# lucidrains/voicebox-pytorch

Hardware: AMD Instinct MI355X
Metric: mel-frames/sec train-step (fwd+bwd+allreduce+clip+Adam) (higher is better)
Workload: dtype f16/bf16 (fp16 forward operands, bf16 backward operands, fp32 accumulate/master); 1 GPU; VoiceBox dim 512 depth 12 heads 16 unconditional, 8x1024 frames per GPU, train; global_batch=8, seq_len=1024, parallelism=dp1

## Files before the change

include/vbx.h:

```cpp
#ifndef VBX_H
#define VBX_H
#include <stddef.h>
#include <stdint.h>

#ifdef __cplusplus
extern "C" {
#endif

#define VBX_VERSION 1

enum { VBX_OK = 0, VBX_EINVAL = -1, VBX_EUNSUPPORTED = -2, VBX_EWORKSPACE = -3 };

int vbx_version(void);
const char* vbx_last_error(void);
int vbx_check_device(int dev);

enum { VBX_GEMM_NT = 0, VBX_GEMM_NN = 1, VBX_GEMM_TN = 2 };

enum {
  VBX_EPI_BF16 = 0,
  VBX_EPI_F32 = 1,
  VBX_EPI_QKV = 2,
  VBX_EPI_GEGLU = 3,
  VBX_EPI_SPLITK = 4,
// ... 352 lines not shown
  float* dcond;
  int dropout;
  unsigned long long drop_seed;
  const float* ada_table;
  const int* ada_counter;
  int ada_slot;
  int ada_stride;
} vbx_io;

size_t vbx_model_wpack_bytes(const vbx_model* m);
size_t vbx_model_act_bytes(const vbx_model* m);
int vbx_model_pack_weights(const vbx_model* m, void* stream);
int vbx_model_adaln_factors(const vbx_model* m, const float** dada, const float** temb, long* w_off, void** dst_f16);
long vbx_model_sq_partials(const vbx_model* m, long* ranges );
int vbx_model_adam_segments(const vbx_model* m, long n_flat, vbx_adam_seg* out, int max_segs, long* total_blocks);
int vbx_model_forward(const vbx_model* m, const vbx_io* io, void* stream);
int vbx_model_adaln_table(const vbx_model* m, const float* temb, int n, float* ada, void* stream);
int vbx_model_backward_head(const vbx_model* m, const vbx_io* io, const float* gscale, void* stream);
int vbx_model_backward_layer(const vbx_model* m, const vbx_io* io, int layer, void* stream);
int vbx_model_backward_embed(const vbx_model* m, const vbx_io* io, void* stream);
int vbx_wgrad_overlap(int on);
int vbx_wgrad_overlap_forks(void);
int vbx_wgrad_overlap_delay(float side_us, float main_us);

void* vbx_model_debug_ptr(const vbx_model* m, const char* name, int layer);

int vbx_split3_f16(const float* src, long rows, int K, long ld, void* dst_f16, int Kp, void* stream);
int vbx_pack_weight3(const float* src, int src_rows, int src_cols, void* dst_f16, int dst_rows, int dst_cols, int rowmap, int F,
                     void* stream);
int vbx_qknorm_rope_f32(const float* raw, int B, int H, int Np, float qk_scale, const float* q_gamma, const float* k_gamma,
                        const float* rot_cos, const float* rot_sin, float* q32, float* k32, float* v32, void* q16, void* k16,
                        void* qb, void* kb, void* v_bf16, void* v16, float* q_rnorm, float* k_rnorm,
                        float q16_scale ,
                        void* stream);
int vbx_attn_fwd_f32(const float* q, const float* k, const float* v, const uint8_t* mask, float* out32, void* out16, void* out_bf16,
                     float* lse, int B, int H, int Np, float scale, void* stream);
int vbx_attn_fwd_f32_dropout(const float* q, const float* k, const float* v, const uint8_t* mask, float* out32, void* out16,
                             void* out_bf16, float* lse, int B, int H, int Np, float scale, const void* bits_rm, float p, void* stream);
int vbx_geglu_f32(const float* h1, float* g32, void* g16, void* g_bf16, void* h1_bf16, long M, int Fp, void* stream);
int vbx_adaln_proj_f32(const float* temb, const float* w, const float* bias, float* ada, int B, int Th, int J, int group, void* stream);
size_t vbx_model_precise_wpack_bytes(const vbx_model* m);
size_t vbx_model_precise_scratch_bytes(const vbx_model* m);
int vbx_model_pack_weights_precise(const vbx_model* m, void* stream);

typedef struct {
  char label[24];
// ... 14 lines not shown
```

voicebox-pytorch_amd/_lib.py:

```python
import ctypes as C
import os

_HERE = os.path.dirname(os.path.abspath(__file__))
LIB_PATH = os.environ.get("VBX_LIB_PATH") or os.path.join(_HERE, "lib", "libvbx_hip.so")

P, I, L, F = C.c_void_p, C.c_int, C.c_long, C.c_float

VBX_GEMM_NT, VBX_GEMM_NN, VBX_GEMM_TN = 0, 1, 2
VBX_EPI_BF16, VBX_EPI_F32, VBX_EPI_QKV, VBX_EPI_GEGLU, VBX_EPI_SPLITK, VBX_EPI_GELU = 0, 1, 2, 3, 4, 5
VBX_GEMM_KERNEL_GEMM5 = 5


class GemmDesc(C.Structure):
    _fields_ = [
        ("mode", I), ("epilogue", I), ("M", I), ("N", I), ("K", I), ("lda", I), ("ldb", I), ("ldc", I),
        ("A", P), ("B", P), ("C", P), ("bias", P), ("resid", P), ("C2", P), ("splits", I),
        ("Np", I), ("H", I), ("qk_scale", F), ("q_gamma", P), ("k_gamma", P), ("rot_cos", P), ("rot_sin", P),
        ("q16", P), ("k16", P), ("qb", P), ("kb", P), ("v", P), ("q_rnorm", P), ("k_rnorm", P), ("f16", I), ("v16", P), ("C3", P),
        ("q_prescale", F),
    ]


_PROTOS = {
    "vbx_version": [],
    "vbx_check_device": [I],
    "vbx_gemm": [C.POINTER(GemmDesc), P],
    "vbx_gemm_select": [I],
    "vbx_gemm_route": [C.POINTER(GemmDesc)],
    "vbx_gemm5_cu_limit": [I],
    "vbx_prof_enable": [I],
    "vbx_wgrad_overlap": [I],
    "vbx_wgrad_overlap_forks": [],
    "vbx_wgrad_overlap_delay": [F, F],
    "vbx_gemm_tn_splitk_grouped": [C.POINTER(GemmDesc), I, P],
    "vbx_splitk_reduce": [P, I, I, I, P, I, I, I, I, I, I, P],
    "vbx_rmsnorm_fwd": [P, P, P, L, P, P, I, I, I, I, I, P],
    "vbx_rmsnorm_bwd_chunks": [I],
    "vbx_rmsnorm_bwd": [P, P, L, P, P, P, P, P, P, I, I, I, I, I, P],
    "vbx_attn_fwd": [P, P, P, P, P, P, P, I, I, I, F, P],
    "vbx_attn_bwd": [P, P, P, P, P, P, P, I, P, P, P, P, P, P, I, I, I, I, F, P, P],
    "vbx_attn_bwd_fused": [P, P, P, P, P, P, P, I, P, P, P, P, P, P, P, P, P, F, P, I, P, I, I, I, F, P, P],
    "vbx_attn_bwd_select": [I],
    "vbx_attn_bwd_variant": [],
    "vbx_dropout_bits_words": [I],
    "vbx_attn_dropout_bits": [P, P, I, I, C.c_ulonglong, C.c_uint, F, P],
    "vbx_dropout_rows": [P, P, L, I, I, C.c_ulonglong, C.c_uint, F, P],
    "vbx_attn_fwd_dropout": [P, P, P, P, P, P, P, I, I, I, F, P, F, P],
    "vbx_attn_bwd_dropout": [P, P, P, P, P, P, P, I, P, P, P, P, P, P, I, I, I, I, F, P, P, F, P],
    "vbx_attn_bwd_fused_tiles": [I],
    "vbx_attn_bwd_fused_dropout": [P, P, P, P, P, P, P, I, P, P, P, P, P, P, P, P, P, F, P, I, P, I, I, I, F, P, P, P, F, P],
    "vbx_qknorm_rope_bwd": [P, P, P, P, P, P, P, P, P, P, F, P, I, P, I, I, I, F, P],
    "vbx_qknorm_rope_bwd_gpart_rows": [I],
    "vbx_pack_embed_input": [P, P, P, P, P, I, I, I, P],
    "vbx_pack_embed_input_text": [P, P, P, P, P, P, I, P, I, L, P, P, I, I, I, P],
    "vbx_cond_emb_bwd": [P, I, P, I, P, L, P, I, I, I, P],
    "vbx_proj_in_kp": [I],
# ... 170 lines not shown
```

voicebox-pytorch_amd/csrc/runtime.hip:

```cpp
#include "common.hpp"
#include "wgrad_overlap_plan.hpp"
#include <stdlib.h>
#include <algorithm>
#include <string.h>
#include <string>
#include <vector>

namespace {

inline size_t al256(size_t x) { return (x + 255) & ~(size_t)255; }

struct Carver {
  char* base;
  size_t off = 0;
  explicit Carver(void* b) : base((char*)b) {}
  template <class T>
  T* take(size_t n) {
    off = al256(off);
    T* p = base ? (T*)(base + off) : nullptr;
    off += n * sizeof(T);
    return p;
  }
};

struct Dims {
  int B, N, R, Np, D, H, I, F, Fp, Th, L, ks, J, E, Ke, Din;
  int Lc, Kp, Do, Dop;
  long M, M0;
// ... 282 lines not shown
    if (!g_prof.on) return;
    if (g_prof.recs.size() >= 8192) return;
    hipStreamCaptureStatus cs = hipStreamCaptureStatusNone;
    if (hipStreamIsCapturing(st, &cs) != hipSuccess || cs != hipStreamCaptureStatusNone) return;
    ProfRec r{label, nullptr, nullptr};
    if (hipEventCreate(&r.e0) != hipSuccess || hipEventCreate(&r.e1) != hipSuccess) return;
    (void)hipEventRecord(r.e0, st);
    idx = (int)g_prof.recs.size();
    g_prof.recs.push_back(r);
  }
  ~ProfScope() {
    if (idx >= 0) (void)hipEventRecord(g_prof.recs[idx].e1, st);
  }
};

#define CK(x)                 \
  do {                        \
    int rc__ = (x);           \
    if (rc__ != 0) return rc__; \
  } while (0)

struct WgoSide {
  hipStream_t st = nullptr;
  hipEvent_t ev[wgrad_overlap::EV_N] = {};
};
int g_wgo_on = -1;
float g_wgo_delay[2] = {0.f, 0.f};
int g_wgo_forks = 0;
bool wgo_enabled() {
  if (g_wgo_on < 0) {
    const char* e = getenv("VBX_WGRAD_OVERLAP");
    g_wgo_on = e ? (atoi(e) != 0) : 1;
  }
  return g_wgo_on != 0;
}
WgoSide* wgo_side(bool create) {
  static WgoSide* sides[64] = {};
  int dev = 0;
  if (hipGetDevice(&dev) != hipSuccess || dev < 0 || dev >= 64) return nullptr;
  if (sides[dev] || !create) return sides[dev];
  WgoSide* s = new WgoSide;
  int least = 0, greatest = 0;
  const char* pe = getenv("VBX_WGRAD_OVERLAP_PRIORITY");
  const bool low = !(pe && !strcmp(pe, "default"));
  bool ok = hipDeviceGetStreamPriorityRange(&least, &greatest) == hipSuccess &&
            hipStreamCreateWithPriority(&s->st, hipStreamNonBlocking, low ? least : 0) == hipSuccess;
  for (int i = 0; ok && i < wgrad_overlap::EV_N; i++) ok = hipEventCreateWithFlags(&s->ev[i], hipEventDisableTiming) == hipSuccess;
  if (!ok) {
    for (auto e : s->ev) if (e) (void)hipEventDestroy(e);
    if (s->st) (void)hipStreamDestroy(s->st);
    delete s;
    (void)hipGetLastError();
    return nullptr;
  }
  return sides[dev] = s;
}
bool capturing(hipStream_t st) {
  hipStreamCaptureStatus cs = hipStreamCaptureStatusNone;
  return hipStreamIsCapturing(st, &cs) != hipSuccess || cs != hipStreamCaptureStatusNone;
}
int wgo_sync(WgoSide* sd, hipStream_t main_st, wgrad_overlap::Point p, int l, int L) {
  if (!sd) return 0;
  const wgrad_overlap::Sync s = wgrad_overlap::sync_at(p, l, L);
  if (s.kind == wgrad_overlap::SYNC_NONE) return 0;
  hipStream_t st = s.stream == wgrad_overlap::MAIN ? main_st : sd->st;
  const hipError_t e = s.kind == wgrad_overlap::SYNC_RECORD ? hipEventRecord(sd->ev[s.ev], st) : hipStreamWaitEvent(st, sd->ev[s.ev], 0);
  VBX_REQUIRE(e == hipSuccess, "weight-gradient overlap: event %s failed (%s)", s.kind == wgrad_overlap::SYNC_RECORD ? "record" : "wait",
              hipGetErrorString(e));
  return 0;
}
struct WgoGuard {
  WgoSide* sd = nullptr;
  bool forked = false, ok = false;
  int done(int rc) { ok = rc == 0; return rc; }
  ~WgoGuard() {
    if (forked && !ok && sd) (void)hipStreamSynchronize(sd->st);
  }
};
bool defers(const vbx_model* m) { return m->defer_reduce && !m->gateloop && !m->unet && (m->plain_norm || m->adaln_factors); }
struct { const void* act = nullptr; int dxb = 0, dqkv = 0; } g_last_copy;

int check_model(const vbx_model* m) {
  VBX_REQUIRE(m && m->params && m->off && m->wpack && m->act && m->rot_cos && m->rot_sin, "vbx_model: null field");
  VBX_REQUIRE(m->D % 64 == 0 && m->D <= 2048, "vbx_model: dim must be a multiple of 64 and <= 2048 (got %d)", m->D);
  VBX_REQUIRE(m->H > 0 && m->H % 2 == 0, "vbx_model: heads must be even (dim_head is fixed at 64)");
  VBX_REQUIRE(m->Th % 8 == 0 && m->L > 0 && m->B > 0 && m->N > 0 && m->R >= 0 && m->F > 0, "vbx_model: bad dims");
  VBX_REQUIRE(m->ksize >= 1 && m->ksize <= 31 && (m->ksize & 1), "vbx_model: conv_pos_embed_kernel_size must be odd and <= 31 (got %d)", m->ksize);
  VBX_REQUIRE(m->E >= 0 && m->E % 8 == 0 && (m->E == 0 || (m->V1 > 0 && !m->stack_only)), "vbx_model: bad dim_cond_emb / table size");
  const long DT = (long)m->D * m->Th;
  for (int l = 0; l < m->L; l++) {
    const long* o = m->off + VBX_NG + (long)l * VBX_NL;
    if (m->plain_norm) continue;
    VBX_REQUIRE(o[VBX_L_B1W] == o[VBX_L_G1W] + DT && o[VBX_L_G2W] == o[VBX_L_B1W] + DT && o[VBX_L_B2W] == o[VBX_L_G2W] + DT,
                "vbx_model: adaLN weights of layer %d are not contiguous in (g1,b1,g2,b2) order", l);
    VBX_REQUIRE(o[VBX_L_B1B] == o[VBX_L_G1B] + m->D && o[VBX_L_G2B] == o[VBX_L_B1B] + m->D && o[VBX_L_B2B] == o[VBX_L_G2B] + m->D,
                "vbx_model: adaLN biases of layer %d are not contiguous in (g1,b1,g2,b2) order", l);
  }
  for (int l = 0; l < m->L && m->gateloop; l++) {
    const long* o = m->off + VBX_NG + (long)l * VBX_NL;
    VBX_REQUIRE(o[VBX_L_GLLNB] == o[VBX_L_GLLNW] + m->D,
                "vbx_model: GateLoop post-LayerNorm weight and bias of layer %d are not contiguous", l);
  }
// ... 102 lines not shown
      CK(vbx_adaln_proj_f32(temb, P + o[VBX_L_G1W], P + o[VBX_L_G1B], ada + (size_t)l * n * 4 * d.D, n, d.Th, 4 * d.D, 4 * d.D, stream));
    }
    return 0;
  }
  return vbx_adaln_proj_fwd(temb, w.adah, w.bada, ada, n, d.Th, d.J, 4 * d.D, stream);
}

extern "C" int vbx_model_forward(const vbx_model* m, const vbx_io* io, void* stream) {
  CK(check_model(m));
  VBX_REQUIRE(io && io->x, "vbx_model_forward: null io field");
  VBX_REQUIRE(m->stack_only ? ((m->plain_norm || io->cond) && io->pred && !io->target) : (io->cond && (io->times || io->ada_table)),
              "vbx_model_forward: null io field");
  VBX_REQUIRE(!io->target || (io->loss_mask && io->loss), "vbx_model_forward: target needs loss_mask and loss");
  VBX_REQUIRE((io->attn_mask == nullptr) == (io->attn_mask_p == nullptr), "vbx_model_forward: attn_mask and attn_mask_p go together");
  hipStream_t st = (hipStream_t)stream;
  const Dims d = dims_of(m);
  WPack w;
  carve_wpack(m, w);
  Acts a;
  carve_acts(m, a);
  const float* P = m->params;
  const long* G = m->off;
  const bool tr = m->training != 0;

  if (m->precise) {
    std::vector<VbxPreciseLayer> pl(d.L);
    for (int l = 0; l < d.L; l++) {
      const ALayer& y = a.layer[l];
      pl[l] = VbxPreciseLayer{y.hn1, y.q16, y.k16, y.qb, y.kb, y.v, y.vh, y.oh, y.o, y.hn2, y.gh, y.g, tr ? y.h1 : nullptr,
                              y.qrn, y.krn, y.lse, w.layer[l].b1, y.hg, y.glp, y.gls, tr ? y.glh : nullptr, (unsigned*)y.dbr, (unsigned*)y.dbc};
    }
    VbxPreciseActs pa{a.four, a.pre, a.temb, a.ada, a.e, a.pred, a.per_b, a.xs.data(), pl.data(), a.embed_in, a.embed_inh, a.hf};
    return vbx_forward_precise(m, io, &pa, stream);
  }

  if (m->stack_only) {
    CK(vbx_stack_input(io->x, d.R ? P + G[VBX_P_REG] : nullptr, a.xs[0], d.B, d.N, d.R, d.D, stream));
    if (!m->plain_norm) CK(vbx_adaln_proj_fwd(io->cond, w.adah, w.bada, a.ada, d.B, d.Th, d.J, 4 * d.D, stream));
  } else {
  if (io->ada_table) {
    VBX_REQUIRE(!tr && io->ada_counter && io->ada_stride >= 1,
                "vbx_model_forward: ada_table is an inference-only input and needs ada_counter and ada_stride >= 1");
    CK(vbx_ada_select(a.ada, d.L, d.B, 4 * d.D, io->ada_table, io->ada_counter, io->ada_stride, io->ada_slot, stream));
  } else {
  CK(vbx_time_embed_fwd(io->times, P + G[VBX_P_SINW], P + G[VBX_P_T1W], P + G[VBX_P_T1B], a.four, a.pre, a.temb, d.B, d.D,
                        d.Th, stream));
  CK(vbx_adaln_proj_fwd(a.temb, w.adah, w.bada, a.ada, d.B, d.Th, d.J, 4 * d.D, stream));
  }
  if (d.Lc) {
    CK(vbx_proj_in_embed(io->x, io->cond, w.pinh, P + G[VBX_P_PINB], io->cond_mask, io->drop_mask, io->null_cond, a.embed_inh,
                         a.embed_in, a.xcb, d.B, d.N, d.Lc, d.D, d.E, stream));
    if (d.E) {
      VBX_REQUIRE(io->cond_ids && io->T > 0, "vbx_model_forward: a text-conditioned model needs cond_ids");
      CK(vbx_embed_text_cols(io->drop_mask, io->cond_ids, io->T, P + G[VBX_P_CEMB], d.E, io->null_id, a.embed_inh, a.embed_in, d.B,
                             d.N, d.D, d.Ke, stream));
    }
  } else if (d.E) {
    VBX_REQUIRE(io->cond_ids && io->T > 0, "vbx_model_forward: a text-conditioned model needs cond_ids");
    CK(vbx_pack_embed_input_text(io->x, io->cond, io->cond_mask, io->drop_mask, io->null_cond, io->cond_ids, io->T,
                                 P + G[VBX_P_CEMB], d.E, io->null_id, a.embed_inh, a.embed_in, d.B, d.N, d.Din, stream));
  } else {
    CK(vbx_pack_embed_input(io->x, io->cond, io->cond_mask, a.embed_inh, a.embed_in, d.B, d.N, d.Din, stream));
  }
  CK(gemm_nt(a.embed_inh, d.Ke, w.embh, d.Ke, (int)d.M0, d.D, d.Ke, VBX_EPI_F32, a.e, d.D, P + G[VBX_P_EMBB], nullptr,
             nullptr, nullptr, st));
  CK(vbx_convpos_fwd(a.e, P + G[VBX_P_CONVW], P + G[VBX_P_CONVB], io->attn_mask, d.R ? P + G[VBX_P_REG] : nullptr, a.xs[0],
                     d.B, d.N, d.R, d.D, d.ks, stream));
  }

  for (int l = 0; l < d.L; l++) {
    const long* o = m->off + VBX_NG + (long)l * VBX_NL;
    const ALayer& y = a.layer[l];
    const float* ada_l = a.ada + (size_t)l * d.B * 4 * d.D;
    const int S = m->gateloop ? 3 : 2;
    float* x0 = layer_input(m, a, l);
    float* x_in = m->gateloop ? a.xs[S * l + 1] : x0;
    float* x_mid = a.xs[S * l + S - 1];
    float* x_out = a.xs[S * l + S];
    if (m->unet && l >= d.L / 2) {
      CK(vbx_unet_cat(a.xs[S * l], a.xs[S * (d.L - 1 - l)], m->skip_scale, a.cat16, nullptr, d.M, d.D, stream));
      CK(gemm_nt(a.cat16, 2 * d.D, w.layer[l].skwh, 2 * d.D, (int)d.M, d.D, 2 * d.D, VBX_EPI_F32, x0, d.D, P + o[VBX_L_SKB], nullptr,
                 nullptr, nullptr, st));
    }
    if (m->gateloop) {
      CK(vbx_rmsnorm_fwd(x0, P + o[VBX_L_GLG], nullptr, 0, y.hg, y.hgh, d.B, d.Np, 0, d.Np, d.D, stream));
      CK(gemm_nt(y.hgh, d.D, w.layer[l].glwh, d.D, (int)d.M, 3 * d.D, d.D, VBX_EPI_F32, y.glp, 3 * d.D, nullptr, nullptr, nullptr,
                 nullptr, st));
      CK(vbx_gateloop_scan_fwd(y.glp, y.gls, tr ? y.glh : nullptr, d.B, d.Np, d.D, stream));
      CK(vbx_layernorm_fwd(y.gls, P + o[VBX_L_GLLNW], P + o[VBX_L_GLLNB], x0, x_in, d.M, d.D, 1e-5f, stream));
    }
// ... 43 lines not shown
  }
  float* pred = io->pred ? io->pred : a.pred;
  CK(gemm_nt(a.hfh, d.D, w.predh, d.D, (int)d.M0, d.Do, d.D, VBX_EPI_F32, pred, d.Do, nullptr, nullptr, nullptr, nullptr, st));
  if (io->target) CK(vbx_masked_mse_fwd(pred, io->target, io->loss_mask, a.per_b, io->loss, d.B, d.N, d.Do, stream));
  return 0;
}

extern "C" int vbx_model_backward_head(const vbx_model* m, const vbx_io* io, const float* gscale, void* stream) {
  CK(check_model(m));
  VBX_REQUIRE(m->training && m->grads && io && io->target && (m->stack_only || io->loss_mask),
              "vbx_model_backward_head: needs a training forward");
  hipStream_t st = (hipStream_t)stream;
  const Dims d = dims_of(m);
  WPack w;
  carve_wpack(m, w);
  Acts a;
  carve_acts(m, a);
  const float* P = m->params;
  float* Gd = m->grads;
  const long* G = m->off;
  WgoGuard guard;
  guard.sd = capturing(st) ? nullptr : wgo_side(false);
  guard.forked = guard.sd != nullptr;
  CK(wgo_sync(guard.sd, st, wgrad_overlap::PT_HEAD_BEGIN, -1, d.L));
  u16* const dxb = defers(m) ? a.copy[wgrad_overlap::BUF_DXB][wgrad_overlap::dxb_read_copy(d.L - 1)] : a.dxb;
  g_last_copy.act = m->act; g_last_copy.dxb = (int)(dxb != a.dxb ? wgrad_overlap::dxb_read_copy(d.L - 1) : 0);
  if (m->stack_only) {
    CK(vbx_pack_weight(io->target, (int)d.M0, d.D, a.dhn, nullptr, (int)d.M0, d.D, 0, 0, stream));
  } else {
    const float* pred = io->pred ? io->pred : a.pred;
    if (d.Dop != d.Do)
      CK(vbx_masked_mse_bwd_ld(a.pred, d.Dop, io->target, io->loss_mask, a.per_b, gscale, a.dpb, d.B, d.N, d.Do, stream));
    else
      CK(vbx_masked_mse_bwd(pred, io->target, io->loss_mask, a.per_b, gscale, nullptr, a.dpb, d.B, d.N, d.Do, stream));
    CK(wgrad(a.dpb, d.Dop, a.hf, d.D, d.Dop, d.D, d.M0, a.slabs, Gd + G[VBX_P_PREDW], d.Do, d.D, 0, 0, st));
    CK(gemm_nn_bf16(a.dpb, d.Dop, w.pred, d.D, (int)d.M0, d.D, d.Dop, a.dhn, d.D, st));
  }
  if (hipMemsetAsync(a.dx, 0, (size_t)d.M * d.D * sizeof(float), st) != hipSuccess ||
      hipMemsetAsync(dxb, 0, (size_t)d.M * d.D * sizeof(u16), st) != hipSuccess) {
    vbx_set_error("vbx_model_backward_head: memset failed");
    return VBX_EINVAL;
  }
  CK(vbx_rmsnorm_bwd(a.xs[(m->gateloop ? 3 : 2) * d.L], P + G[VBX_P_FNG], 0, a.dhn, nullptr, a.dx, dxb, a.npart, nullptr, d.B, d.Np, d.R, d.N, d.D,
                     stream));
  CK(vbx_reduce_norm_partials(a.npart, a.tmp2d, 0, d.B, vbx_rmsnorm_bwd_chunks(d.N), d.D, 1, stream));
  CK(vbx_sum_rows_f32(a.tmp2d, 1, d.D, Gd + G[VBX_P_FNG], d.D, 0, stream));
  return guard.done(0);
}

struct SqLayout { long off[4], per_layer; };
static SqLayout sq_layout(const Dims& d) {
  SqLayout q;
  const long n[4] = {vbx_splitk_reduce_blocks(d.D, d.Fp), vbx_splitk_reduce_blocks(2 * d.Fp, d.D), vbx_splitk_reduce_blocks(d.D, d.I),
                     vbx_splitk_reduce_blocks(3 * d.I, d.D)};
  q.off[0] = 0;
  for (int i = 1; i < 4; i++) q.off[i] = q.off[i - 1] + n[i - 1];
  q.per_layer = q.off[3] + n[3];
  return q;
}
extern "C" long vbx_model_sq_partials(const vbx_model* m, long* ranges) {
  if (check_model(m) != 0) return 0;
  const Dims d = dims_of(m);
  if (ranges) {
    for (int l = 0; l < d.L; l++) {
      const long* o = m->off + VBX_NG + (long)l * VBX_NL;
      const long lo[4] = {o[VBX_L_QKVW], o[VBX_L_OUTW], o[VBX_L_FF1W], o[VBX_L_FF2W]};
      const long sz[4] = {3L * d.I * d.D, (long)d.D * d.I, 2L * d.F * d.D, (long)d.D * d.F};
      for (int i = 0; i < 4; i++) {
        if (i && lo[i] < lo[i - 1] + sz[i - 1]) return 0;
// ... 123 lines not shown
  float* const npart2 = a.npart2 + rr * a.np_stride;
  float* const cpart = a.cpart + rr * a.cp_stride;
  float* const gpart = a.gpart + rr * a.gp_stride;
  float* const csl = pl.defer ? a.cs_layers + rr * a.cs_stride : a.cs_scratch;
  vbx_skr_jobs wj{};
  WgradGroup wgg;
  WgradGroup* wgp = group_wgrad() ? &wgg : nullptr;
  const int gs = wgp ? wgrad_splits3(d) : 0;
  namespace wgo = wgrad_overlap;
  auto copy_of = [&](wgo::Buf b) { return pl.defer ? a.copy[b][wgo::write_copy(b, l)] : a.copy[b][0]; };
  u16* const dxb_in = pl.defer ? a.copy[wgo::BUF_DXB][wgo::dxb_read_copy(l)] : a.dxb;
  u16* const dxb_out = copy_of(wgo::BUF_DXB);
  u16* const dh1 = copy_of(wgo::BUF_DH1);
  u16* const dqkv = copy_of(wgo::BUF_DQKV);
  u16* dxb_attn = wgp ? copy_of(wgo::BUF_DXB2) : dxb_in;
  g_last_copy.act = m->act; g_last_copy.dxb = pl.defer ? wgo::write_copy(wgo::BUF_DXB, l) : 0; g_last_copy.dqkv = pl.defer ? wgo::write_copy(wgo::BUF_DQKV, l) : 0;
  const bool cap = capturing(st);
  const bool fork = pl.defer && wgp && wgo_enabled() && !g_prof.on && !cap;
  WgoGuard guard;
  guard.sd = cap ? nullptr : wgo_side(fork);
  VBX_REQUIRE(!fork || guard.sd, "vbx_model_backward_layer: could not create the weight-gradient side stream");
  if (fork && g_wgo_delay[1] > 0.f) CK(vbx_stream_delay(g_wgo_delay[1], stream));
  CK(wgo_sync(guard.sd, st, wgo::PT_LAYER_BEGIN, l, d.L));
  float* const slabs = fork ? a.slabs_side : a.slabs;
  const size_t sfl = a.slab_floats;
  const SqLayout sql = sq_layout(d);
  float* const sqb = m->sq_partials ? m->sq_partials + (long)l * sql.per_layer : nullptr;
  auto sq_at = [&](int i) { return sqb ? sqb + sql.off[i] : nullptr; };

  { ProfScope ps("dgrad ff_out", st); CK(gemm_nn_bf16(dxb_in, d.D, wl.w2, d.Fp, M, d.Fp, d.D, a.dg, d.Fp, st)); }
  CK(wgrad(dxb_in, d.D, y.g, d.Fp, d.D, d.Fp, d.M, slabs, Gd + o[VBX_L_FF2W], d.D, d.F, 0, 0, st, &wj, wgp, gs, sq_at(0)));
  if (drop_on && m->ff_dropout > 0.f)
    CK(vbx_dropout_rows(nullptr, a.dg, d.M, d.Fp, d.Fp, io->drop_seed, 2u * l + 1u, m->ff_dropout, stream));
  CK(vbx_geglu_bwd_colsum(y.h1, a.dg, dh1, M, d.Fp, csl, stream));
  { ProfScope ps("dgrad ff_in", st); CK(gemm_nn_bf16(dh1, 2 * d.Fp, wl.w1, d.D, M, d.D, 2 * d.Fp, a.dhn, d.D, st)); }
  CK(wgrad(dh1, 2 * d.Fp, y.hn2, d.D, 2 * d.Fp, d.D, d.M, slabs + sfl, Gd + o[VBX_L_FF1W], 2 * d.F, d.D, 1, d.F, st, &wj, wgp, gs, sq_at(1)));
  CK(vbx_rmsnorm_bwd(x_mid, g2, gstride, a.dhn, a.dx, a.dx, dxb_attn, npart, cpart, d.B, d.Np, 0, d.Np, d.D, stream));

  { ProfScope ps("dgrad to_out", st); CK(gemm_nn_bf16(dxb_attn, d.D, wl.out, d.I, M, d.I, d.D, a.dO, d.I, st)); }
  CK(wgrad(dxb_attn, d.D, y.o, d.I, d.D, d.I, d.M, slabs + 2 * sfl, Gd + o[VBX_L_OUTW], d.D, d.I, 0, 0, st, &wj, wgp, gs, sq_at(2)));
  { ProfScope ps("bwd attention", st);
    CK(vbx_attn_bwd_fused_dropout(y.q16, y.k16, y.qb, y.kb, y.v, attn_mask_p, y.oh, 1, a.dO, y.lse, a.delta, y.qrn, y.krn, q_gamma, k_gamma,
                                  m->rot_cos, m->rot_sin, m->qk_norm ? 8.0f : 0.0f, dqkv, 3 * d.I, gpart, d.B, d.H, d.Np, m->attn_scale,
                                  a.attn_scratch, drop_on ? y.dbr : nullptr, y.dbc, m->attn_dropout, stream)); }
  { ProfScope ps("dgrad to_qkv", st); CK(gemm_nn_bf16(dqkv, 3 * d.I, wl.qkv, d.D, M, d.D, 3 * d.I, a.dhn, d.D, st)); }
  CK(wgrad(dqkv, 3 * d.I, y.hn1, d.D, 3 * d.I, d.D, d.M, slabs + 3 * sfl, Gd + o[VBX_L_QKVW], 3 * d.I, d.D, 0, 0, st, &wj, wgp, gs, sq_at(3)));

  if (fork) {
    hipStream_t side = guard.sd->st;
    CK(wgo_sync(guard.sd, st, wgo::PT_FORK, l, d.L));
    guard.forked = true;
    g_wgo_forks++;
    CK(wgo_sync(guard.sd, st, wgo::PT_SIDE_BEGIN, l, d.L));
    if (g_wgo_delay[0] > 0.f) CK(vbx_stream_delay(g_wgo_delay[0], side));
    if (wgg.n) CK(vbx_gemm_tn_splitk_grouped(wgg.d, wgg.n, side));
    CK(wgo_sync(guard.sd, st, wgo::PT_SIDE_GEMM_DONE, l, d.L));
    if (wj.n) CK(vbx_splitk_reduce_multi(&wj, side));
    CK(wgo_sync(guard.sd, st, wgo::PT_SIDE_REDUCE_DONE, l, d.L));
  } else {
    if (wgg.n) { ProfScope ps("wgrad (4 GEMMs)", st); CK(vbx_gemm_tn_splitk_grouped(wgg.d, wgg.n, stream)); }
    if (wj.n) { ProfScope ps("wgrad slab reduce", st); CK(vbx_splitk_reduce_multi(&wj, stream)); }
  }
  CK(vbx_rmsnorm_bwd(x_in, g1, gstride, a.dhn, a.dx, a.dx, dxb_out, npart2, nullptr, d.B, d.Np, 0, d.Np, d.D, stream));

  vbx_mr_jobs jb{};
  if (!pl.defer) {
    layer_reduce_jobs(m, d, a, pl, l, 0, jb);
    CK(vbx_multi_reduce(&jb, stream));
  } else if (l == 0) {
    ProfScope ps("partials reduce (all)", st);
    for (int ll = d.L - 1; ll >= 0; ll--) {
      layer_reduce_jobs(m, d, a, pl, ll, ll, jb);
      if (jb.n + 8 > VBX_MR_MAX || ll == 0) {
        CK(vbx_multi_reduce(&jb, stream));
        jb.n = 0;
      }
    }
  }

  if (m->gateloop) CK(backward_gateloop(m, d, w, a, l, stream));
  if (m->unet) CK(backward_unet(m, d, w, a, l, stream));
  if (m->plain_norm) return guard.done(0);
  if (pl.ada_all) {
    if (l == 0) {
      ProfScope ps("adaLN dtemb (all)", st);
      CK(vbx_adaln_dtemb_all(w.adah, a.dada, a.dtemb, a.ada_scratch, d.L, d.B, d.Th, 4 * d.D, stream));
    }
    return guard.done(0);
  }
  return guard.done(vbx_adaln_proj_bwd(m->stack_only ? io->cond : a.temb, w.adah + (size_t)l * 4 * d.D * d.Th, dada_l,
                            m->adaln_factors ? nullptr : Gd + o[VBX_L_G1W], Gd + o[VBX_L_G1B], a.dtemb,
                            a.ada_scratch, d.B, d.Th, 4 * d.D, l == d.L - 1 ? 0 : 1, stream));
}

extern "C" int vbx_model_backward_embed(const vbx_model* m, const vbx_io* io, void* stream) {
  CK(check_model(m));
  VBX_REQUIRE(m->training && m->grads && io && (m->stack_only ? io->dx != nullptr : io->times != nullptr),
              "vbx_model_backward_embed: needs a training forward");
  hipStream_t st = (hipStream_t)stream;
  const Dims d = dims_of(m);
  WPack w;
  carve_wpack(m, w);
  Acts a;
  carve_acts(m, a);
  const float* P = m->params;
  float* Gd = m->grads;
  const long* G = m->off;
// ... 103 lines not shown
  carve_acts(m, a);
  if (dada) *dada = a.dada;
  if (temb) *temb = a.temb;
  for (int l = 0; l < d.L; l++) {
    if (w_off) w_off[l] = (m->off + VBX_NG + (long)l * VBX_NL)[VBX_L_G1W];
    if (dst_f16) dst_f16[l] = w.adah + (size_t)l * 4 * d.D * d.Th;
  }
  return d.L;
}

extern "C" int vbx_wgrad_overlap(int on) {
  VBX_REQUIRE(on == 0 || on == 1, "vbx_wgrad_overlap: 0 in line, 1 on the side stream");
  g_wgo_on = on;
  return 0;
}
extern "C" int vbx_wgrad_overlap_forks(void) { return g_wgo_forks; }
extern "C" int vbx_wgrad_overlap_delay(float side_us, float main_us) {
  VBX_REQUIRE(side_us >= 0.f && side_us <= 2000.f && main_us >= 0.f && main_us <= 2000.f, "vbx_wgrad_overlap_delay: 0 .. 2000 us each");
  g_wgo_delay[0] = side_us;
  g_wgo_delay[1] = main_us;
  return 0;
}

extern "C" int vbx_prof_enable(int on) {
  for (auto& r : g_prof.recs) { (void)hipEventDestroy(r.e0); (void)hipEventDestroy(r.e1); }
  g_prof.recs.clear();
  g_prof.on = on != 0;
  return 0;
}
extern "C" int vbx_prof_collect(vbx_prof_entry* out, int max_entries) {
  VBX_REQUIRE(out && max_entries > 0, "vbx_prof_collect: bad args");
  g_prof.on = false;
  int n = 0;
  for (auto& r : g_prof.recs) {
    float ms = 0.f;
    if (hipEventSynchronize(r.e1) != hipSuccess || hipEventElapsedTime(&ms, r.e0, r.e1) != hipSuccess) continue;
    int k = 0;
    for (; k < n; k++)
      if (!strncmp(out[k].label, r.label, sizeof(out[k].label) - 1)) break;
    if (k == n) {
      if (n == max_entries) continue;
      memset(&out[n], 0, sizeof(out[n]));
      strncpy(out[n].label, r.label, sizeof(out[n].label) - 1);
      n++;
    }
    out[k].calls++;
// ... 31 lines not shown
```

Measured before the change: 939,500 mel-frames/s.

## Overlap forward adaLN, head wgrad, memsets and partial reductions on side stream

Extends the side-stream overlap beyond layer weight gradients. The forward time embedding and adaLN projections now run on the side stream while the embed branch runs on main. In backward, the head's to_pred wgrad, the dx/dxb memsets and the final-norm gamma reductions move to the side stream, and deferred per-layer partial reductions are spread across layers on the side stream instead of being done all at layer 0. This is meant to hide small serial kernels behind the main chain, at the cost of extra event syncs, added dependency tracking and a global map of reduction state keyed by activation buffer.

```diff
diff --git a/include/vbx.h b/include/vbx.h
--- a/include/vbx.h
+++ b/include/vbx.h
@@ -398,6 +398,14 @@
 int vbx_wgrad_overlap(int on);
 int vbx_wgrad_overlap_forks(void);
 int vbx_wgrad_overlap_delay(float side_us, float main_us);
+#define VBX_STEP_OVERLAP_FWD 1
+#define VBX_STEP_OVERLAP_HEAD 2
+#define VBX_STEP_OVERLAP_PARTIALS 4
+#define VBX_STEP_OVERLAP_MEMSET 8
+int vbx_step_overlap(int on);
+int vbx_step_overlap_parts(int parts);
+int vbx_step_overlap_forks(void);
+int vbx_step_overlap_plan_forks(int L, int forward);
 
 void* vbx_model_debug_ptr(const vbx_model* m, const char* name, int layer);
 
diff --git a/voicebox-pytorch_amd/_lib.py b/voicebox-pytorch_amd/_lib.py
--- a/voicebox-pytorch_amd/_lib.py
+++ b/voicebox-pytorch_amd/_lib.py
@@ -32,6 +32,10 @@
     "vbx_wgrad_overlap": [I],
     "vbx_wgrad_overlap_forks": [],
     "vbx_wgrad_overlap_delay": [F, F],
+    "vbx_step_overlap": [I],
+    "vbx_step_overlap_parts": [I],
+    "vbx_step_overlap_forks": [],
+    "vbx_step_overlap_plan_forks": [I, I],
     "vbx_gemm_tn_splitk_grouped": [C.POINTER(GemmDesc), I, P],
     "vbx_splitk_reduce": [P, I, I, I, P, I, I, I, I, I, I, P],
     "vbx_rmsnorm_fwd": [P, P, P, L, P, P, I, I, I, I, I, P],
diff --git a/voicebox-pytorch_amd/csrc/runtime.hip b/voicebox-pytorch_amd/csrc/runtime.hip
--- a/voicebox-pytorch_amd/csrc/runtime.hip
+++ b/voicebox-pytorch_amd/csrc/runtime.hip
@@ -1,9 +1,11 @@
 #include "common.hpp"
+#include "step_overlap_plan.hpp"
 #include "wgrad_overlap_plan.hpp"
 #include <stdlib.h>
 #include <algorithm>
 #include <string.h>
 #include <string>
+#include <unordered_map>
 #include <vector>
 
 namespace {
@@ -332,7 +334,7 @@
 
 struct WgoSide {
   hipStream_t st = nullptr;
-  hipEvent_t ev[wgrad_overlap::EV_N] = {};
+  hipEvent_t ev[step_overlap::EV_N] = {};
 };
 int g_wgo_on = -1;
 float g_wgo_delay[2] = {0.f, 0.f};
@@ -355,7 +357,7 @@
   const bool low = !(pe && !strcmp(pe, "default"));
   bool ok = hipDeviceGetStreamPriorityRange(&least, &greatest) == hipSuccess &&
             hipStreamCreateWithPriority(&s->st, hipStreamNonBlocking, low ? least : 0) == hipSuccess;
-  for (int i = 0; ok && i < wgrad_overlap::EV_N; i++) ok = hipEventCreateWithFlags(&s->ev[i], hipEventDisableTiming) == hipSuccess;
+  for (int i = 0; ok && i < step_overlap::EV_N; i++) ok = hipEventCreateWithFlags(&s->ev[i], hipEventDisableTiming) == hipSuccess;
   if (!ok) {
     for (auto e : s->ev) if (e) (void)hipEventDestroy(e);
     if (s->st) (void)hipStreamDestroy(s->st);
@@ -388,6 +390,30 @@
   }
 };
 bool defers(const vbx_model* m) { return m->defer_reduce && !m->gateloop && !m->unet && (m->plain_norm || m->adaln_factors); }
+int g_sto_on = -1;
+int g_sto_parts = -1;
+int g_sto_forks = 0;
+int sto_parts() {
+  if (g_sto_on < 0) {
+    const char* e = getenv("VBX_STEP_OVERLAP");
+    g_sto_on = e ? (atoi(e) != 0) : 1;
+  }
+  if (g_sto_parts < 0) {
+    const char* e = getenv("VBX_STEP_OVERLAP_PARTS");
+    g_sto_parts = e ? (atoi(e) & step_overlap::PART_ALL) : step_overlap::kDefaultParts;
+  }
+  return g_sto_on && wgo_enabled() ? g_sto_parts : 0;
+}
+int sto_sync(WgoSide* sd, hipStream_t main_st, step_overlap::Point p, int l, int L, int parts) {
+  if (!sd) return 0;
+  const step_overlap::Sync s = step_overlap::sync_at(p, l, L, parts);
+  if (s.kind == wgrad_overlap::SYNC_NONE) return 0;
+  hipStream_t st = s.stream == wgrad_overlap::MAIN ? main_st : sd->st;
+  const hipError_t e = s.kind == wgrad_overlap::SYNC_RECORD ? hipEventRecord(sd->ev[s.ev], st) : hipStreamWaitEvent(st, sd->ev[s.ev], 0);
+  VBX_REQUIRE(e == hipSuccess, "step overlap: event %s failed (%s)", s.kind == wgrad_overlap::SYNC_RECORD ? "record" : "wait", hipGetErrorString(e));
+  return 0;
+}
+std::unordered_map<const void*, int> g_sto_reduced;
 struct { const void* act = nullptr; int dxb = 0, dqkv = 0; } g_last_copy;
 
 int check_model(const vbx_model* m) {
@@ -536,6 +562,17 @@
   const float* P = m->params;
   const long* G = m->off;
   const bool tr = m->training != 0;
+  namespace sto = step_overlap;
+  const bool fwd_cap = tr ? capturing(st) : true;
+  const int fwd_parts = (tr && !fwd_cap && !m->stack_only && !m->precise && !m->gateloop && !m->unet && !io->ada_table && !g_prof.on) ? sto_parts() : 0;
+  const bool fwd_fork = sto::has(fwd_parts, sto::PART_FWD);
+  WgoGuard guard;
+  guard.sd = fwd_cap ? nullptr : wgo_side(fwd_fork);
+  VBX_REQUIRE(!fwd_fork || guard.sd, "vbx_model_forward: could not create the side stream");
+  if (fwd_parts) {
+    if (fwd_fork && g_wgo_delay[1] > 0.f) CK(vbx_stream_delay(g_wgo_delay[1], stream));
+    CK(sto_sync(guard.sd, st, sto::PT_FWD_BEGIN_JOIN, -1, d.L, fwd_parts));
+  }
 
   if (m->precise) {
     std::vector<VbxPreciseLayer> pl(d.L);
@@ -557,9 +594,18 @@
                 "vbx_model_forward: ada_table is an inference-only input and needs ada_counter and ada_stride >= 1");
     CK(vbx_ada_select(a.ada, d.L, d.B, 4 * d.D, io->ada_table, io->ada_counter, io->ada_stride, io->ada_slot, stream));
   } else {
+  void* const ada_stream = fwd_fork ? (void*)guard.sd->st : stream;
+  if (fwd_fork) {
+    CK(sto_sync(guard.sd, st, sto::PT_FWD_BEGIN, -1, d.L, fwd_parts));
+    guard.forked = true;
+    g_sto_forks++;
+    CK(sto_sync(guard.sd, st, sto::PT_FWD_SIDE_BEGIN, -1, d.L, fwd_parts));
+    if (g_wgo_delay[0] > 0.f) CK(vbx_stream_delay(g_wgo_delay[0], ada_stream));
+  }
   CK(vbx_time_embed_fwd(io->times, P + G[VBX_P_SINW], P + G[VBX_P_T1W], P + G[VBX_P_T1B], a.four, a.pre, a.temb, d.B, d.D,
-                        d.Th, stream));
-  CK(vbx_adaln_proj_fwd(a.temb, w.adah, w.bada, a.ada, d.B, d.Th, d.J, 4 * d.D, stream));
+                        d.Th, ada_stream));
+  CK(vbx_adaln_proj_fwd(a.temb, w.adah, w.bada, a.ada, d.B, d.Th, d.J, 4 * d.D, ada_stream));
+  if (fwd_fork) CK(sto_sync(guard.sd, st, sto::PT_FWD_SIDE_DONE, -1, d.L, fwd_parts));
   }
   if (d.Lc) {
     CK(vbx_proj_in_embed(io->x, io->cond, w.pinh, P + G[VBX_P_PINB], io->cond_mask, io->drop_mask, io->null_cond, a.embed_inh,
@@ -580,6 +626,10 @@
              nullptr, nullptr, st));
   CK(vbx_convpos_fwd(a.e, P + G[VBX_P_CONVW], P + G[VBX_P_CONVB], io->attn_mask, d.R ? P + G[VBX_P_REG] : nullptr, a.xs[0],
                      d.B, d.N, d.R, d.D, d.ks, stream));
+  }
+  if (fwd_fork) {
+    CK(sto_sync(guard.sd, st, sto::PT_FWD_JOIN, -1, d.L, fwd_parts));
+    guard.forked = false;
   }
 
   for (int l = 0; l < d.L; l++) {
@@ -669,9 +719,29 @@
   WgoGuard guard;
   guard.sd = capturing(st) ? nullptr : wgo_side(false);
   guard.forked = guard.sd != nullptr;
+  namespace sto = step_overlap;
+  const bool cap = capturing(st);
+  const int parts = (defers(m) && !m->stack_only && group_wgrad() && !g_prof.on && !cap) ? sto_parts() : 0;
+  const bool fork = sto::has(parts, sto::PART_HEAD), zero_side = sto::has(parts, sto::PART_HEAD | sto::PART_MEMSET);
+  if (fork) {
+    guard.sd = wgo_side(true);
+    guard.forked = true;
+    VBX_REQUIRE(guard.sd, "vbx_model_backward_head: could not create the side stream");
+    if (g_wgo_delay[1] > 0.f) CK(vbx_stream_delay(g_wgo_delay[1], stream));
+  }
+  hipStream_t const side = fork ? guard.sd->st : st;
+  g_sto_reduced[m->act] = d.L;
   CK(wgo_sync(guard.sd, st, wgrad_overlap::PT_HEAD_BEGIN, -1, d.L));
   u16* const dxb = defers(m) ? a.copy[wgrad_overlap::BUF_DXB][wgrad_overlap::dxb_read_copy(d.L - 1)] : a.dxb;
   g_last_copy.act = m->act; g_last_copy.dxb = (int)(dxb != a.dxb ? wgrad_overlap::dxb_read_copy(d.L - 1) : 0);
+  auto zero_dx = [&](hipStream_t on) {
+    if (hipMemsetAsync(a.dx, 0, (size_t)d.M * d.D * sizeof(float), on) != hipSuccess ||
+        hipMemsetAsync(dxb, 0, (size_t)d.M * d.D * sizeof(u16), on) != hipSuccess) {
+      vbx_set_error("vbx_model_backward_head: memset failed");
+      return (int)VBX_EINVAL;
+    }
+    return 0;
+  };
   if (m->stack_only) {
     CK(vbx_pack_weight(io->target, (int)d.M0, d.D, a.dhn, nullptr, (int)d.M0, d.D, 0, 0, stream));
   } else {
@@ -680,18 +750,33 @@
       CK(vbx_masked_mse_bwd_ld(a.pred, d.Dop, io->target, io->loss_mask, a.per_b, gscale, a.dpb, d.B, d.N, d.Do, stream));
     else
       CK(vbx_masked_mse_bwd(pred, io->target, io->loss_mask, a.per_b, gscale, nullptr, a.dpb, d.B, d.N, d.Do, stream));
-    CK(wgrad(a.dpb, d.Dop, a.hf, d.D, d.Dop, d.D, d.M0, a.slabs, Gd + G[VBX_P_PREDW], d.Do, d.D, 0, 0, st));
+    if (fork) {
+      CK(sto_sync(guard.sd, st, sto::PT_HEAD_FORK, -1, d.L, parts));
+      g_sto_forks++;
+      CK(sto_sync(guard.sd, st, sto::PT_HEAD_SIDE_BEGIN, -1, d.L, parts));
+      if (g_wgo_delay[0] > 0.f) CK(vbx_stream_delay(g_wgo_delay[0], side));
+      if (zero_side) {
+        CK(zero_dx(side));
+        CK(sto_sync(guard.sd, st, sto::PT_HEAD_SIDE_ZERO, -1, d.L, parts));
+      }
+    }
+    CK(wgrad(a.dpb, d.Dop, a.hf, d.D, d.Dop, d.D, d.M0, fork ? a.slabs_side : a.slabs, Gd + G[VBX_P_PREDW], d.Do, d.D, 0, 0, side));
     CK(gemm_nn_bf16(a.dpb, d.Dop, w.pred, d.D, (int)d.M0, d.D, d.Dop, a.dhn, d.D, st));
   }
-  if (hipMemsetAsync(a.dx, 0, (size_t)d.M * d.D * sizeof(float), st) != hipSuccess ||
-      hipMemsetAsync(dxb, 0, (size_t)d.M * d.D * sizeof(u16), st) != hipSuccess) {
-    vbx_set_error("vbx_model_backward_head: memset failed");
-    return VBX_EINVAL;
-  }
+  if (zero_side) CK(sto_sync(guard.sd, st, sto::PT_HEAD_ZERO_JOIN, -1, d.L, parts));
+  else CK(zero_dx(st));
   CK(vbx_rmsnorm_bwd(a.xs[(m->gateloop ? 3 : 2) * d.L], P + G[VBX_P_FNG], 0, a.dhn, nullptr, a.dx, dxb, a.npart, nullptr, d.B, d.Np, d.R, d.N, d.D,
                      stream));
-  CK(vbx_reduce_norm_partials(a.npart, a.tmp2d, 0, d.B, vbx_rmsnorm_bwd_chunks(d.N), d.D, 1, stream));
-  CK(vbx_sum_rows_f32(a.tmp2d, 1, d.D, Gd + G[VBX_P_FNG], d.D, 0, stream));
+  if (fork) {
+    CK(sto_sync(guard.sd, st, sto::PT_HEAD_NORM, -1, d.L, parts));
+    CK(sto_sync(guard.sd, st, sto::PT_HEAD_SIDE_NORM, -1, d.L, parts));
+  }
+  CK(vbx_reduce_norm_partials(a.npart, a.tmp2d, 0, d.B, vbx_rmsnorm_bwd_chunks(d.N), d.D, 1, side));
+  CK(vbx_sum_rows_f32(a.tmp2d, 1, d.D, Gd + G[VBX_P_FNG], d.D, 0, side));
+  if (fork) {
+    CK(sto_sync(guard.sd, st, sto::PT_HEAD_SIDE_DONE, -1, d.L, parts));
+    CK(sto_sync(guard.sd, st, sto::PT_HEAD_SIDE_JOIN, -1, d.L, parts));
+  }
   return guard.done(0);
 }
 
@@ -861,6 +946,12 @@
   VBX_REQUIRE(!fork || guard.sd, "vbx_model_backward_layer: could not create the weight-gradient side stream");
   if (fork && g_wgo_delay[1] > 0.f) CK(vbx_stream_delay(g_wgo_delay[1], stream));
   CK(wgo_sync(guard.sd, st, wgo::PT_LAYER_BEGIN, l, d.L));
+  namespace sto = step_overlap;
+  const int parts = sto_parts();
+  CK(sto_sync(guard.sd, st, sto::PT_LAYER0_BEGIN, l, d.L, parts));
+  auto red = g_sto_reduced.find(m->act);
+  if (red == g_sto_reduced.end() || l == d.L - 1) red = g_sto_reduced.insert_or_assign(m->act, d.L).first;
+  int& reduced_from = red->second;
   float* const slabs = fork ? a.slabs_side : a.slabs;
   const size_t sfl = a.slab_floats;
   const SqLayout sql = sq_layout(d);
@@ -892,6 +983,19 @@
     g_wgo_forks++;
     CK(wgo_sync(guard.sd, st, wgo::PT_SIDE_BEGIN, l, d.L));
     if (g_wgo_delay[0] > 0.f) CK(vbx_stream_delay(g_wgo_delay[0], side));
+    if (sto::has(parts, sto::PART_PARTIALS) && reduced_from > l + 1) {
+      vbx_mr_jobs sj{};
+      for (int ll = reduced_from - 1; ll > l; ll--) {
+        layer_reduce_jobs(m, d, a, pl, ll, ll, sj);
+        if (sj.n + 8 > VBX_MR_MAX || ll == l + 1) {
+          CK(vbx_multi_reduce(&sj, side));
+          sj.n = 0;
+        }
+      }
+      reduced_from = l + 1;
+      g_sto_forks++;
+      CK(sto_sync(guard.sd, st, sto::PT_SIDE_PARTIALS_DONE, l, d.L, parts));
+    }
     if (wgg.n) CK(vbx_gemm_tn_splitk_grouped(wgg.d, wgg.n, side));
     CK(wgo_sync(guard.sd, st, wgo::PT_SIDE_GEMM_DONE, l, d.L));
     if (wj.n) CK(vbx_splitk_reduce_multi(&wj, side));
@@ -908,7 +1012,7 @@
     CK(vbx_multi_reduce(&jb, stream));
   } else if (l == 0) {
     ProfScope ps("partials reduce (all)", st);
-    for (int ll = d.L - 1; ll >= 0; ll--) {
+    for (int ll = reduced_from - 1; ll >= 0; ll--) {
       layer_reduce_jobs(m, d, a, pl, ll, ll, jb);
       if (jb.n + 8 > VBX_MR_MAX || ll == 0) {
         CK(vbx_multi_reduce(&jb, stream));
@@ -922,6 +1026,7 @@
   if (m->plain_norm) return guard.done(0);
   if (pl.ada_all) {
     if (l == 0) {
+      if (reduced_from < d.L) CK(sto_sync(guard.sd, st, sto::PT_DTEMB_BEGIN, l, d.L, sto::PART_PARTIALS));
       ProfScope ps("adaLN dtemb (all)", st);
       CK(vbx_adaln_dtemb_all(w.adah, a.dada, a.dtemb, a.ada_scratch, d.L, d.B, d.Th, 4 * d.D, stream));
     }
@@ -1071,6 +1176,22 @@
   return 0;
 }
 
+extern "C" int vbx_step_overlap(int on) {
+  VBX_REQUIRE(on == 0 || on == 1, "vbx_step_overlap: 0 in line, 1 beside the main chain");
+  g_sto_on = on;
+  return 0;
+}
+extern "C" int vbx_step_overlap_parts(int parts) {
+  VBX_REQUIRE(parts >= -1 && parts <= step_overlap::PART_ALL, "vbx_step_overlap_parts: a mask of VBX_STEP_OVERLAP_* bits, or -1 for the default");
+  g_sto_parts = parts < 0 ? step_overlap::kDefaultParts : parts;
+  return 0;
+}
+extern "C" int vbx_step_overlap_forks(void) { return g_sto_forks; }
+extern "C" int vbx_step_overlap_plan_forks(int L, int forward) {
+  const int parts = sto_parts();
+  return forward ? step_overlap::forward_forks(parts) : step_overlap::backward_forks(L, parts);
+}
+
 extern "C" int vbx_prof_enable(int on) {
   for (auto& r : g_prof.recs) { (void)hipEventDestroy(r.e0); (void)hipEventDestroy(r.e1); }
   g_prof.recs.clear();
diff --git a/voicebox-pytorch_amd/csrc/step_overlap_plan.hpp b/voicebox-pytorch_amd/csrc/step_overlap_plan.hpp
--- /dev/null
+++ b/voicebox-pytorch_amd/csrc/step_overlap_plan.hpp
@@ -0,0 +1,228 @@
+#pragma once
+#include <cstring>
+#include <initializer_list>
+
+#include "wgrad_overlap_plan.hpp"
+
+namespace step_overlap {
+
+namespace wgo = wgrad_overlap;
+using wgo::MAIN;
+using wgo::SIDE;
+using wgo::Stream;
+using wgo::SyncKind;
+
+enum Part { PART_FWD = 1, PART_HEAD = 2, PART_PARTIALS = 4, PART_MEMSET = 8, PART_ALL = 15 };
+constexpr int kDefaultParts = PART_FWD | PART_HEAD | PART_PARTIALS | PART_MEMSET;
+
+enum Event {
+  EV_FWD_BEGIN = wgo::EV_N,
+  EV_ADA,
+  EV_HEAD_FORK,
+  EV_HEAD_ZERO,
+  EV_HEAD_NORM,
+  EV_HEAD_DONE,
+  EV_PARTIALS,
+  EV_N
+};
+
+enum Point {
+  PT_FWD_BEGIN_JOIN,
+  PT_FWD_BEGIN,
+  PT_FWD_SIDE_BEGIN,
+  PT_FWD_SIDE_DONE,
+  PT_FWD_JOIN,
+  PT_HEAD_FORK,
+  PT_HEAD_SIDE_BEGIN,
+  PT_HEAD_SIDE_ZERO,
+  PT_HEAD_ZERO_JOIN,
+  PT_HEAD_NORM,
+  PT_HEAD_SIDE_NORM,
+  PT_HEAD_SIDE_DONE,
+  PT_HEAD_SIDE_JOIN,
+  PT_LAYER0_BEGIN,
+  PT_SIDE_PARTIALS_DONE,
+  PT_DTEMB_BEGIN,
+};
+struct Sync {
+  SyncKind kind;
+  Stream stream;
+  int ev;
+};
+constexpr Sync kNoSync{wgo::SYNC_NONE, MAIN, EV_N};
+constexpr bool has(int parts, int p) { return (parts & p) == p; }
+constexpr Sync sync_at(Point p, int l, int L, int parts) {
+  const bool fwd = has(parts, PART_FWD), head = has(parts, PART_HEAD), zero = has(parts, PART_HEAD | PART_MEMSET);
+  const bool partials = has(parts, PART_PARTIALS) && L >= 2;
+  switch (p) {
+    case PT_FWD_BEGIN_JOIN: return parts ? Sync{wgo::SYNC_WAIT, MAIN, wgo::EV_JOIN} : kNoSync;
+    case PT_FWD_BEGIN: return fwd ? Sync{wgo::SYNC_RECORD, MAIN, EV_FWD_BEGIN} : kNoSync;
+    case PT_FWD_SIDE_BEGIN: return fwd ? Sync{wgo::SYNC_WAIT, SIDE, EV_FWD_BEGIN} : kNoSync;
+    case PT_FWD_SIDE_DONE: return fwd ? Sync{wgo::SYNC_RECORD, SIDE, EV_ADA} : kNoSync;
+    case PT_FWD_JOIN: return fwd ? Sync{wgo::SYNC_WAIT, MAIN, EV_ADA} : kNoSync;
+    case PT_HEAD_FORK: return head ? Sync{wgo::SYNC_RECORD, MAIN, EV_HEAD_FORK} : kNoSync;
+    case PT_HEAD_SIDE_BEGIN: return head ? Sync{wgo::SYNC_WAIT, SIDE, EV_HEAD_FORK} : kNoSync;
+    case PT_HEAD_SIDE_ZERO: return zero ? Sync{wgo::SYNC_RECORD, SIDE, EV_HEAD_ZERO} : kNoSync;
+    case PT_HEAD_ZERO_JOIN: return zero ? Sync{wgo::SYNC_WAIT, MAIN, EV_HEAD_ZERO} : kNoSync;
+    case PT_HEAD_NORM: return head ? Sync{wgo::SYNC_RECORD, MAIN, EV_HEAD_NORM} : kNoSync;
+    case PT_HEAD_SIDE_NORM: return head ? Sync{wgo::SYNC_WAIT, SIDE, EV_HEAD_NORM} : kNoSync;
+    case PT_HEAD_SIDE_DONE: return head ? Sync{wgo::SYNC_RECORD, SIDE, EV_HEAD_DONE} : kNoSync;
+    case PT_HEAD_SIDE_JOIN: return head ? Sync{wgo::SYNC_RECORD, SIDE, wgo::EV_JOIN} : kNoSync;
+    case PT_LAYER0_BEGIN: return head && l == 0 && wgo::last_reader(0, L) < 0 ? Sync{wgo::SYNC_WAIT, MAIN, EV_HEAD_DONE} : kNoSync;
+    case PT_SIDE_PARTIALS_DONE: return partials && l + 1 < L ? Sync{wgo::SYNC_RECORD, SIDE, EV_PARTIALS} : kNoSync;
+    case PT_DTEMB_BEGIN: return partials && l == 0 ? Sync{wgo::SYNC_WAIT, MAIN, EV_PARTIALS} : kNoSync;
+  }
+  return kNoSync;
+}
+constexpr int forward_forks(int parts) { return has(parts, PART_FWD) ? 1 : 0; }
+constexpr int backward_forks(int L, int parts) { return (has(parts, PART_HEAD) ? 1 : 0) + (has(parts, PART_PARTIALS) ? L - 1 : 0); }
+
+enum ResKind {
+  RES_TIME = 100,
+  RES_ADA,
+  RES_DPB,
+  RES_DX,
+  RES_PARTIALS,
+  RES_TMP2D,
+  RES_DADA,
+  RES_GRAD_SMALL,
+  RES_DTEMB,
+  RES_GRAD_TIME,
+};
+struct Res {
+  int kind, a, b;
+};
+struct Op {
+  enum Type { LAUNCH, SYNC } type;
+  Stream stream;
+  const char* name;
+  int layer;
+  Sync sync;
+  bool is_new;
+  Res reads[10], writes[6];
+  int nr, nw;
+};
+inline Op from_wgo(const wgo::Op& w) {
+  Op o{};
+  o.type = w.type == wgo::Op::SYNC ? Op::SYNC : Op::LAUNCH;
+  o.stream = w.stream; o.name = w.name; o.layer = w.layer;
+  o.sync = Sync{w.sync.kind, w.sync.stream, (int)w.sync.ev};
+  for (int i = 0; i < w.nr; i++) o.reads[o.nr++] = Res{(int)w.reads[i].kind, w.reads[i].a, w.reads[i].b};
+  for (int i = 0; i < w.nw; i++) o.writes[o.nw++] = Res{(int)w.writes[i].kind, w.writes[i].a, w.writes[i].b};
+  return o;
+}
+template <class F>
+inline void put_sync(Point p, int l, int L, int parts, F&& f) {
+  const Sync s = sync_at(p, l, L, parts);
+  if (s.kind == wgo::SYNC_NONE) return;
+  Op o{};
+  o.type = Op::SYNC; o.stream = s.stream; o.name = s.kind == wgo::SYNC_WAIT ? "wait" : "record"; o.layer = l; o.sync = s; o.is_new = true;
+  f(o);
+}
+template <class F>
+inline void put_launch(Stream st, const char* name, int l, std::initializer_list<Res> reads, std::initializer_list<Res> writes, F&& f) {
+  Op o{};
+  o.type = Op::LAUNCH; o.stream = st; o.name = name; o.layer = l;
+  for (const Res& r : reads) o.reads[o.nr++] = r;
+  for (const Res& w : writes) o.writes[o.nw++] = w;
+  f(o);
+}
+
+constexpr Res kActs{wgo::RES_FWD_ACTS, 0, 0}, kTime{RES_TIME, 0, 0}, kAda{RES_ADA, 0, 0}, kDpb{RES_DPB, 0, 0}, kDx{RES_DX, 0, 0};
+constexpr Res kTmp2d{RES_TMP2D, 0, 0}, kDtemb{RES_DTEMB, 0, 0}, kSlabsSide{wgo::RES_SLABS_SIDE, 0, 0}, kSlabsMain{wgo::RES_SLABS_MAIN, 0, 0};
+constexpr Res kGradHead{wgo::RES_GRAD_HEAD, 0, 0}, kGradEmbed{wgo::RES_GRAD_EMBED, 0, 0}, kGradTime{RES_GRAD_TIME, 0, 0};
+constexpr Res partials(int region) { return Res{RES_PARTIALS, region, 0}; }
+constexpr Res dada(int l) { return Res{RES_DADA, l, 0}; }
+constexpr Res grad_small(int l) { return Res{RES_GRAD_SMALL, l, 0}; }
+
+template <class F>
+inline void emit_forward(int L, int parts, F&& f) {
+  const Stream ada_on = has(parts, PART_FWD) ? SIDE : MAIN;
+  put_sync(PT_FWD_BEGIN_JOIN, -1, L, parts, f);
+  put_sync(PT_FWD_BEGIN, -1, L, parts, f);
+  put_sync(PT_FWD_SIDE_BEGIN, -1, L, parts, f);
+  put_launch(ada_on, "time embedding", -1, {}, {kTime}, f);
+  put_launch(ada_on, "adaLN projections", -1, {kTime}, {kAda}, f);
+  put_sync(PT_FWD_SIDE_DONE, -1, L, parts, f);
+  put_launch(MAIN, "embed branch (pack, to_embed, conv)", -1, {}, {kActs}, f);
+  put_sync(PT_FWD_JOIN, -1, L, parts, f);
+  for (int l = 0; l < L; l++) put_launch(MAIN, "forward layer", l, {kAda, kActs}, {kActs}, f);
+  put_launch(MAIN, "final norm, to_pred, loss", -1, {kActs}, {kActs}, f);
+}
+
+template <class F>
+inline void emit_head(int L, int parts, F&& f) {
+  const bool head = has(parts, PART_HEAD), zero = has(parts, PART_HEAD | PART_MEMSET);
+  const Res dxb{wgo::RES_BUF, wgo::BUF_DXB, wgo::dxb_read_copy(L - 1)};
+  wgo::emit_sync(wgo::PT_HEAD_BEGIN, -1, L, [&](const wgo::Op& o) { f(from_wgo(o)); });
+  put_launch(MAIN, "mse backward", -1, {kActs}, {kDpb}, f);
+  put_sync(PT_HEAD_FORK, -1, L, parts, f);
+  put_sync(PT_HEAD_SIDE_BEGIN, -1, L, parts, f);
+  if (zero) put_launch(SIDE, "memsets (dx, dxb)", -1, {}, {kDx, dxb}, f);
+  put_sync(PT_HEAD_SIDE_ZERO, -1, L, parts, f);
+  put_launch(head ? SIDE : MAIN, "to_pred wgrad + reduce", -1, {kDpb, kActs}, {head ? kSlabsSide : kSlabsMain, kGradHead}, f);
+  put_launch(MAIN, "dgrad to_pred", -1, {kDpb}, {}, f);
+  if (!zero) put_launch(MAIN, "memsets (dx, dxb)", -1, {}, {kDx, dxb}, f);
+  put_sync(PT_HEAD_ZERO_JOIN, -1, L, parts, f);
+  put_launch(MAIN, "final norm backward", -1, {kActs}, {kDx, dxb, partials(0)}, f);
+  put_sync(PT_HEAD_NORM, -1, L, parts, f);
+  put_sync(PT_HEAD_SIDE_NORM, -1, L, parts, f);
+  put_launch(head ? SIDE : MAIN, "final norm gamma: reduce partials", -1, {partials(0)}, {kTmp2d}, f);
+  put_launch(head ? SIDE : MAIN, "final norm gamma: sum rows", -1, {kTmp2d}, {kGradHead}, f);
+  put_sync(PT_HEAD_SIDE_DONE, -1, L, parts, f);
+  put_sync(PT_HEAD_SIDE_JOIN, -1, L, parts, f);
+}
+
+template <class F>
+inline void emit_layer(int l, int L, int parts, F&& f) {
+  const bool partials_side = has(parts, PART_PARTIALS);
+  put_sync(PT_LAYER0_BEGIN, l, L, parts, f);
+  wgo::emit_layer(l, L, [&](const wgo::Op& w) {
+    Op o = from_wgo(w);
+    if (w.type == wgo::Op::LAUNCH && w.stream == MAIN) {
+      const bool norm = !strncmp(w.name, "norm backward", 13);
+      if (norm) { o.reads[o.nr++] = kAda; o.reads[o.nr++] = kDx; o.writes[o.nw++] = kDx; }
+      if (norm || !strcmp(w.name, "GEGLU backward") || !strcmp(w.name, "attention backward")) o.writes[o.nw++] = partials(l);
+    }
+    f(o);
+    if (w.type == wgo::Op::SYNC && w.point == wgo::PT_SIDE_BEGIN && partials_side && l + 1 < L) {
+      put_launch(SIDE, "partials reduce", l + 1, {partials(l + 1)}, {dada(l + 1), grad_small(l + 1)}, f);
+      put_sync(PT_SIDE_PARTIALS_DONE, l, L, parts, f);
+    }
+  });
+  if (l != 0) return;
+  for (int ll = L - 1; ll >= 0; ll--)
+    if (ll == 0 || !partials_side) put_launch(MAIN, "partials reduce", ll, {partials(ll)}, {dada(ll), grad_small(ll)}, f);
+  put_sync(PT_DTEMB_BEGIN, 0, L, parts, f);
+  Op o{};
+  o.type = Op::LAUNCH; o.stream = MAIN; o.name = "adaLN dtemb (all)"; o.layer = -1;
+  o.reads[o.nr++] = dada(0);
+  o.writes[o.nw++] = kDtemb;
+  f(o);
+}
+
+template <class F>
+inline void emit_embed(int L, int parts, F&& f) {
+  (void)parts;
+  put_launch(MAIN, "conv backward + finalize", -1, {kDx, kActs}, {kGradEmbed}, f);
+  wgo::emit_embed(L, [&](const wgo::Op& w) {
+    if (w.type == wgo::Op::SYNC) {
+      put_launch(MAIN, "time MLP backward", -1, {kDtemb, kTime}, {kGradTime}, f);
+    }
+    f(from_wgo(w));
+  });
+}
+
+template <class F>
+inline void emit_backward(int L, int parts, F&& f) {
+  emit_head(L, parts, f);
+  for (int l = L - 1; l >= 0; l--) emit_layer(l, L, parts, f);
+  emit_embed(L, parts, f);
+}
+template <class F>
+inline void emit_step(int L, int parts, F&& f) {
+  emit_forward(L, parts, f);
+  emit_backward(L, parts, f);
+}
+
+}
```

New measurement: 945,800 mel-frames/s, median of 6. No clear change (+0.7%).
